# nianticlabs/simplerecon

Hardware: AMD Instinct MI355X
Metric: depth frames/sec (640x480, 7 src views, 64 planes) (higher is better)
Workload: dtype f32

## Files before the change

### include/simplerecon_hip.h

```cpp
#ifndef SIMPLERECON_HIP_H_
#define SIMPLERECON_HIP_H_

#include <stddef.h>
#include <stdint.h>

#ifdef __cplusplus
extern "C" {
#endif

#define SR_OK 0
#define SR_ERR_INVALID_ARGUMENT 1
#define SR_ERR_UNSUPPORTED 2
#define SR_ERR_WORKSPACE_TOO_SMALL 3
#define SR_ERR_HIP_BASE 1000

enum {
  SR_OPT_MLP_SPLIT = 0, SR_OPT_WINO_SPLIT, SR_OPT_WINO_XCD, SR_OPT_WINO_NT, SR_OPT_WINO_KSPLIT, SR_OPT_CONV_WINO,
  SR_OPT_CONV_TILE, SR_OPT_CONV_KSPLIT, SR_OPT_PW_NT, SR_OPT_PW_KS, SR_OPT_PT_CFG, SR_OPT_PT_KS, SR_OPT_DOT_LDS,
  SR_OPT_DOT_LDS_G, SR_OPT_DOT_LDS_CULL, SR_OPT_DOT_LDS_CAP, SR_OPT_UPSAMPLE_QUAD, SR_OPT_POOL_STREAM,
  SR_OPT_MLP_TILE,
  SR_OPT_COUNT
};
int sr_option_count(void);
const char* sr_option_name(int id);
int sr_option_id(const char* name);
int sr_option_get(int id, int* value);
int sr_option_set(int id, int value, int* previous );
int sr_option_default(int id, int* value);

int sr_abi_version(void);

const char* sr_target_arch(void);


size_t sr_volume_workspace_bytes(int B, int K, int C, int h, int w);

int sr_volume_prepare(const float* src, const float* K_src, const float* T_src_cur,
                      const float* T_cur_src, int B, int K, int C, int h, int w, void* workspace,
                      size_t workspace_bytes, void* stream);

int sr_dot_volume_sweep(const float* cur, const float* invK_cur, const float* planes, int64_t ps_b,
                        int64_t ps_d, int64_t ps_y, int64_t ps_x, int B, int K, int C, int h, int w,
                        int D, float* out_cv, int64_t cv_sb, int64_t cv_sd, int64_t cv_sp,
// ... 39 lines not shown
                      int h, int w, int D, float* out_cv, int64_t cv_sb, int64_t cv_sd,
                      int64_t cv_sp, float* out_lowest, uint8_t* out_mask, void* workspace,
                      size_t workspace_bytes, void* stream);

int sr_warp_features_fwd(const float* src, const float* K_src, const float* T_src_cur,
                         const float* invK_cur, const float* planes, int64_t ps_b, int64_t ps_d,
                         int64_t ps_y, int64_t ps_x, int B, int K, int C, int h, int w, int Dp,
                         float* out_world, float* out_depths, float* out_warped, float* out_mask,
                         float* out_pix, void* workspace, size_t workspace_bytes, void* stream);

size_t sr_mlp_volume_workspace_bytes(int B, int K, int C, int h, int w, int hidden);

int sr_mlp_pack_weights(const float* W1, const float* b1, const float* W2, const float* b2,
                        const float* W3, const float* b3, int hidden, int B, int K, int C, int h, int w,
                        void* workspace, size_t workspace_bytes, void* stream);

int sr_mlp_volume_sweep(const float* cur, const float* invK_cur, const float* planes, int64_t ps_b,
                        int64_t ps_d, int64_t ps_y, int64_t ps_x, float leaky_slope, int B, int K,
                        int C, int h, int w, int D, float* out_cv, int64_t cv_sb, int64_t cv_sd,
                        int64_t cv_sp, float* out_lowest, uint8_t* out_mask, void* workspace,
                        size_t workspace_bytes, void* stream);

int sr_mlp_volume_tile_shape(int h, int w, int* th, int* tw);

int sr_mlp_volume_fwd(const float* cur, const float* src, const float* K_src, const float* T_src_cur,
                      const float* T_cur_src, const float* invK_cur, const float* planes, int64_t ps_b,
                      int64_t ps_d, int64_t ps_y, int64_t ps_x, const float* W1, const float* b1,
                      const float* W2, const float* b2, const float* W3, const float* b3, int hidden,
                      float leaky_slope, int B, int K, int C, int h, int w, int D, float* out_cv,
                      int64_t cv_sb, int64_t cv_sd, int64_t cv_sp, float* out_lowest, uint8_t* out_mask,
                      int reserve_cus, void* workspace, size_t workspace_bytes, void* stream);


size_t sr_conv_packed_weight_floats(int Cout, int Cin, int ksize);

int sr_conv_pack_weights(const float* weight, int Cout, int Cin, int ksize, float* packed, void* stream);

int sr_conv2d_nhwc_fwd(const float* in, int64_t in_batch_stride, int in_pix_stride,
                       const float* packed_weight, const float* bias, const float* residual,
                       int64_t res_batch_stride, int res_pix_stride, float* out,
                       int64_t out_batch_stride, int out_pix_stride, int B, int H, int W, int Cin,
                       int Cout, int ksize, int stride, float leaky_slope, void* stream);

int sr_conv2d_replicate_nhwc_fwd(const float* in, int64_t in_batch_stride, int in_pix_stride,
                                 const float* packed_weight, const float* bias, const float* residual,
                                 int64_t res_batch_stride, int res_pix_stride, float* out,
// ... 422 lines not shown
```

### simplerecon_amd/_lib.py

```python
import contextlib
import ctypes as C
import os

import torch

_HERE = os.path.dirname(os.path.abspath(__file__))
LIB_PATH = os.environ.get("SR_HIP_LIBRARY") or os.path.join(_HERE, "libsimplerecon_hip.so")
ABI_VERSION = 3

_lib = None

_p = C.c_void_p
_i = C.c_int
_i64 = C.c_int64
_f = C.c_float
_sz = C.c_size_t

SIGNATURES = {
    "sr_abi_version": (_i, []),
    "sr_option_count": (_i, []),
    "sr_option_name": (C.c_char_p, [_i]),
    "sr_option_id": (_i, [C.c_char_p]),
    "sr_option_get": (_i, [_i, C.POINTER(C.c_int)]),
    "sr_option_set": (_i, [_i, _i, C.POINTER(C.c_int)]),
# ... 20 lines not shown
    "sr_conv16_wgrad_nhwc": (_i, [_p, _i64, _i, _p, _i64, _i, _p, _i, _i, _i, _i, _i, _i, _i, _i, _p, _sz, _p]),
    "sr_act_bwd_bias16_workspace_bytes": (_sz, [_i64, _i]),
    "sr_act_bwd_bias16_nhwc": (_i, [_p, _i, _p, _p, _p, _i64, _i, _f, _i, _p, _sz, _p]),
    "sr_pw_conv_tiled_workspace_bytes": (_sz, [_i, _i, _i]),
    "sr_pw_conv_tiled_plan": (_i, [_i, _i, _i, _i, _p, _p]),
    "sr_pw_conv_tiled_nhwc_fwd": (_i, [_p, _i, _p, _p, _p, _p, _i, _p, _i, _i, _i, _i, _i, _f, _p, _sz, _p]),
    "sr_pw_conv_supported": (_i, [_i, _i]),
    "sr_pw_conv_plan": (_i, [_i, _i, _i, _i, _p, _p]),
    "sr_pw_conv_nhwc_fwd": (_i, [_p, _i64, _i, _p, _p, _p, _p, _i64, _i, _p, _i64, _i, _i, _i, _i, _i, _f, _p]),
    "sr_backproject_fwd": (_i, [_p, _p, _p, _i, _i, _i, _p]),
    "sr_project3d_fwd": (_i, [_p, _p, _p, _p, _i, _i, _f, _p]),
    "sr_backproject_bwd": (_i, [_p, _p, _p, _i, _i, _i, _p]),
    "sr_project3d_bwd": (_i, [_p, _p, _p, _p, _p, _i, _i, _f, _p]),
    "sr_pose_distance_fwd": (_i, [_p, _p, _i, _p]),
    "sr_camera_rays_fwd": (_i, [_p, _p, _p, _i, _i, _i, _p]),
    "sr_selftest_rcp": (_i, [_p, _p, _p, _i, _p]),
    "sr_warp_features_fwd": (_i, [_p, _p, _p, _p, _p, _i64, _i64, _i64, _i64, _i, _i, _i, _i, _i, _i,
                                  _p, _p, _p, _p, _p, _p, _sz, _p]),
    "sr_mlp_volume_workspace_bytes": (_sz, [_i, _i, _i, _i, _i, _i]),
    "sr_mlp_pack_weights": (_i, [_p, _p, _p, _p, _p, _p, _i, _i, _i, _i, _i, _i, _p, _sz, _p]),
    "sr_mlp_volume_sweep": (_i, [_p, _p, _p, _i64, _i64, _i64, _i64, _f, _i, _i, _i, _i, _i, _i,
                                 _p, _i64, _i64, _i64, _p, _p, _p, _sz, _p]),
    "sr_mlp_volume_tile_shape": (_i, [_i, _i, C.POINTER(C.c_int), C.POINTER(C.c_int)]),
    "sr_mlp_volume_fwd": (_i, [_p, _p, _p, _p, _p, _p, _p, _i64, _i64, _i64, _i64, _p, _p, _p, _p, _p, _p, _i,
                               _f, _i, _i, _i, _i, _i, _i, _p, _i64, _i64, _i64, _p, _p, _i, _p, _sz, _p]),
    "sr_conv_packed_weight_floats": (_sz, [_i, _i, _i]),
    "sr_conv_pack_weights": (_i, [_p, _i, _i, _i, _p, _p]),
    "sr_conv2d_nhwc_fwd": (_i, [_p, _i64, _i, _p, _p, _p, _i64, _i, _p, _i64, _i, _i, _i, _i, _i, _i, _i, _i, _f, _p]),
    "sr_conv2d_replicate_nhwc_fwd": (_i, [_p, _i64, _i, _p, _p, _p, _i64, _i, _p, _i64, _i, _i, _i, _i, _i, _i, _i, _i,
                                          _f, _p]),
    "sr_conv2d_padded_nhwc_fwd": (_i, [_p, _i64, _i, _p, _p, _p, _i64, _i, _p, _i64, _i, _i, _i, _i, _i, _i, _i, _i,
                                       _i, _i, _i, _i, _f, _p]),
    "sr_dwconv3x3_pool_bands": (_i, [_i]),
    "sr_dwconv3x3_nhwc_fwd": (_i, [_p, _i64, _i, _p, _p, _p, _i64, _i, _p, _i, _i, _i, _i, _i, _i, _i, _i, _i, _f,
                                   _p]),
    "sr_add_nhwc_fwd": (_i, [_p, _i64, _i, _p, _i64, _i, _p, _i64, _i, _i, _i, _i, _i, _p]),
    "sr_se_scale_nhwc_fwd": (_i, [_p, _i, _p, _p, _p, _p, _p, _p, _i64, _i, _p, _i64, _i, _p, _i, _i, _i, _i, _i,
                                  _p]),
    "sr_se_gate_fwd": (_i, [_p, _i, _i, _p, _p, _p, _p, _p, _i, _i, _i, _p]),
    "sr_scale_channels_nhwc_fwd": (_i, [_p, _i64, _i, _p, _p, _i64, _i, _i, _i, _i, _i, _p]),
    "sr_dot_volume_bwd_scratch_bytes": (_sz, [_i, _i, _i, _i, _i]),
    "sr_dot_volume_bwd": (_i, [_p, _i64, _i64, _i64, _p, _p, _p, _i64, _i64, _i64, _i64, _i, _i, _i, _i, _i, _i, _p, _p,
                               _p, _sz, _p, _sz, _p]),
    "sr_mlp_volume_bwd_scratch_bytes": (_sz, [_i, _i, _i, _i, _i, _i]),
    "sr_mlp_volume_bwd": (_i, [_p, _i64, _i64, _i64, _p, _p, _p, _i64, _i64, _i64, _i64, _p, _p, _p, _p, _p, _f, _i, _i,
                               _i, _i, _i, _i, _i, _p, _p, _p, _p, _p, _p, _p, _p, _p, _sz, _p, _sz, _p]),
# ... 318 lines not shown
```

### simplerecon_amd/cost_volume.py

```python
import torch
from torch import Tensor, nn

from . import _lib
from .geometry import BackprojectDepth, Project3D
from .networks import MLP


def _autocast_on(device_type):
    try:
        return torch.is_autocast_enabled(device_type)
    except TypeError:
        return torch.is_autocast_enabled()


def _autocast_to_f32(*tensors):
    out = []
    for t in tensors:
        if isinstance(t, Tensor) and t.dtype in (torch.float16, torch.bfloat16) and _autocast_on(t.device.type):
            t = t.float()
        out.append(t)
    return out


class _DotVolumeFunction(torch.autograd.Function):
# ... 332 lines not shown
        lib = _lib.lib()
        vol, lowest, mask = self._alloc_outputs(b, h, w, dev, return_mask)
        if b == 0:
            return vol, lowest, mask
        params = [t.detach() for t in params]
        hidden = params[0].shape[0]
        nws = lib.sr_mlp_volume_workspace_bytes(b, k, c, h, w, hidden)
        ws = self._get_workspace(nws, dev)
        sb, sd, sp = self._volume_strides(vol)
        from . import ops
        cin, d = c * (k + 1) + 10 * k + 4, self.num_depth_bins
        record = lambda: ("sr_mlp_volume_fwd", 2.0 * (cin * hidden + hidden * hidden + hidden) * b * d * h * w, (), None)
        with _lib.SPLIT_GUARD:
            rc = ops._timed(
                dev, record, lib.sr_mlp_volume_fwd,
                _lib.ptr(cur), _lib.ptr(src), _lib.ptr(Ks), _lib.ptr(T), _lib.ptr(Tp), _lib.ptr(invK),
                _lib.ptr(planes), *planes.stride(), *[_lib.ptr(t) for t in params], hidden,
                0.01,
                b, k, c, h, w, d, _lib.ptr(vol), sb, sd, sp, _lib.ptr(lowest),
                _lib.ptr(mask), int(reserve_cus), _lib.ptr(ws), ws.numel(), _lib.stream_ptr(dev))
        _lib.check(rc, "sr_mlp_volume_fwd")
        return vol, lowest, mask

    def to_fast(self) -> "FastFeatureVolumeManager":
        manager = FastFeatureVolumeManager(self.matching_height, self.matching_width,
                                           num_depth_bins=self.num_depth_bins, mlp_channels=self.mlp_channels,
                                           matching_dim_size=self.matching_dim_size,
                                           num_source_views=self.num_source_views)
        manager.to(self.linear_ramp_1d11.device)
        manager.mlp = self.mlp
        manager.volume_memory_format = self.volume_memory_format
        return manager


class FastFeatureVolumeManager(FeatureVolumeManager):

    def warp_features(self, src_feats, src_extrinsics, src_Ks, cur_invK, depth_plane_bdhw, batch_size,
                      num_src_frames, num_feat_channels, uv_scale=None):
        world, depths, warped, mask, pix = self._warp(src_feats, src_extrinsics, src_Ks, cur_invK,
                                                      depth_plane_bdhw, True)
        b, dp = world.shape[:2]
        h, w = self.matching_height, self.matching_width
        world_bkd4hw = world.view(b, 1, dp, 4, h, w).expand(b, num_src_frames, dp, 4, h, w)
        return world_bkd4hw, depths, warped, mask, pix


# ... 20 lines not shown
```

### simplerecon_amd/csrc/sr_mlp_volume.hip

```cpp
#include <stdlib.h>
#include <string.h>

#include "sr_buffer.h"
#include "sr_view.h"

#define SR_HID 128
#define SR_VIEW_SLOTS 24
#define SR_INV_FIXED 20
#define SR_PLANE_CHUNK 8

static inline int sr_mlp_steps_var(int K) { return (SR_VIEW_SLOTS / 2) * K; }
static inline int sr_mlp_steps_inv(int K) { return (SR_INV_FIXED + 3 * K + 1) / 2; }
static inline int sr_mlp_steps1(int K) { return sr_mlp_steps_var(K) + sr_mlp_steps_inv(K); }
#define SR_MLP_STEPS2 65

static inline size_t sr_mlp_packed_floats(int K) { return (size_t)(sr_mlp_steps1(K) + SR_MLP_STEPS2) * 256 + 128 + 4; }

__global__ void sr_mlp_pack_kernel(const float* __restrict__ W1, const float* __restrict__ b1,
                                   const float* __restrict__ W2, const float* __restrict__ b2,
                                   const float* __restrict__ W3, const float* __restrict__ b3,
                                   float* __restrict__ packed, int K, int C) {
  const int steps_var = (SR_VIEW_SLOTS / 2) * K;
  const int steps1 = steps_var + (SR_INV_FIXED + 3 * K + 1) / 2;
  const int Cin = C * (K + 1) + 10 * K + 4;
// ... 46 lines not shown
    } else {
      v = b3[0];
    }
    packed[e] = v;
  }
}


struct SrMlpParams {
  const float* cur;
  const float* src_nhwc;
  const float* invK;
  const float* geom;
  const float* packed;
  SrPlanes planes;
  SrVolumeOut out;
  int B, K, h, w, D;
  int tiles;
  int tiles_x;
  int th_log2, tw_log2;
  int chunk, chunks;
  int vec_store;
  float inv_w, inv_h, slope;
};

__device__ __forceinline__ bool sr_mlp_lane_pixel(const SrMlpParams& p, int tile, int lane, int& y, int& x) {
  if (p.tiles_x) {
    const int ty = tile / p.tiles_x, tx = tile - ty * p.tiles_x;
    const int ly = (ty << p.th_log2) + (lane >> p.tw_log2);
    const int lx = (tx << p.tw_log2) + (lane & ((1 << p.tw_log2) - 1));
    y = min(ly, p.h - 1);
    x = min(lx, p.w - 1);
    return ly < p.h && lx < p.w;
  }
  const int N = p.h * p.w, pix = tile * 64 + lane;
  const int pc = min(pix, N - 1);
  y = pc / p.w;
  x = pc - y * p.w;
  return pix < N;
}

__device__ __forceinline__ void sr_swap_halves(float fa, float fb, float& bP, float& bQ) {
  auto r = __builtin_amdgcn_permlane32_swap(__float_as_uint(fa), __float_as_uint(fb), false, false);
  bP = __uint_as_float(r[0]);
  bQ = __uint_as_float(r[1]);
}

#define SR_MFMA(a, b, c) __builtin_amdgcn_mfma_f32_32x32x2f32((a), (b), (c), 0, 0, 0)

__device__ __forceinline__ void sr_l1_step(f32x16 (&acc)[2][4], const float4 wA, float fa, float fb) {
  float bP, bQ;
  sr_swap_halves(fa, fb, bP, bQ);
  acc[0][0] = SR_MFMA(wA.x, bP, acc[0][0]);
  acc[1][0] = SR_MFMA(wA.x, bQ, acc[1][0]);
  acc[0][1] = SR_MFMA(wA.y, bP, acc[0][1]);
  acc[1][1] = SR_MFMA(wA.y, bQ, acc[1][1]);
  acc[0][2] = SR_MFMA(wA.z, bP, acc[0][2]);
  acc[1][2] = SR_MFMA(wA.z, bQ, acc[1][2]);
  acc[0][3] = SR_MFMA(wA.w, bP, acc[0][3]);
  acc[1][3] = SR_MFMA(wA.w, bQ, acc[1][3]);
}

// ... 29 lines not shown
  const int steps1 = steps_var + (SR_INV_FIXED + 3 * p.K + 1) / 2;
  const float4* gW1 = reinterpret_cast<const float4*>(p.packed);
  const float4* gW1inv = gW1 + (size_t)steps_var * 64;
  const float4* gW2 = gW1 + (size_t)steps1 * 64;
  const float* gW3 = p.packed + (size_t)(steps1 + SR_MLP_STEPS2) * 256;

  for (int i = threadIdx.x; i < 129; i += blockDim.x) lds[i] = gW3[i];
  constexpr int W2_FLOATS = W2_LDS ? SR_MLP_STEPS2 * 256 : 0;
  if (W2_LDS) {
    float4* l4 = reinterpret_cast<float4*>(lds + SR_LDS_W3_FLOATS);
    for (int i = threadIdx.x; i < SR_MLP_STEPS2 * 64; i += blockDim.x) l4[i] = gW2[i];
  }
  if (W1_LDS) {
    float4* l4 = reinterpret_cast<float4*>(lds + SR_LDS_W3_FLOATS + W2_FLOATS);
    for (int i = threadIdx.x; i < steps_var * 64; i += blockDim.x) l4[i] = gW1[i];
  }
  __syncthreads();
  const float4* W1p = W1_LDS ? reinterpret_cast<const float4*>(lds + SR_LDS_W3_FLOATS + W2_FLOATS) : gW1;

  const int N = p.h * p.w;
  const long nunits = (long)p.B * p.tiles * p.chunks;
  constexpr int WPB = 4;
  const int wid = __builtin_amdgcn_readfirstlane(threadIdx.x >> 6);
  long wave0 = (long)blockIdx.x * WPB + wid;
  long nwaves = (long)gridDim.x * WPB;
  long unit_end = nunits;
  if ((gridDim.x & 7) == 0) {
    const long u8 = (nunits + 7) / 8;
    const int xcd = blockIdx.x & 7;
    nwaves = (long)(gridDim.x >> 3) * WPB;
    wave0 = xcd * u8 + (long)(blockIdx.x >> 3) * WPB + wid;
    unit_end = min(nunits, (xcd + 1) * u8);
  }
  const int half = lane >> 5;

  const int rot = (int)max(1L, nwaves / p.chunks);
  for (long unit = wave0; unit < unit_end; unit += nwaves) {
    const long tb = unit / p.chunks;
    const int chunk = (int)((unit % p.chunks + tb / rot) % p.chunks);
    const int tile = (int)(tb % p.tiles);
    const int b = (int)(tb / p.tiles);
    const int j0 = chunk * p.chunk, j1 = min(p.D, j0 + p.chunk);
    int y, x;
    const bool in_image = sr_mlp_lane_pixel(p, tile, lane, y, x);
    const int pc = y * p.w + x;
    const int pix = in_image ? pc : -1;
    const bool active = pix >= 0;
    const float* plane_ptr = p.planes.ptr + b * p.planes.sb + y * p.planes.sy + x * p.planes.sx;
    const float* geom_b = p.geom + (size_t)b * p.K * SR_GEOM_STRIDE;
    const float* src_b = p.src_nhwc + (size_t)b * p.K * N * C;

    float cur[C];
#pragma unroll
    for (int c = 0; c < C; ++c) cur[c] = p.cur[((size_t)b * C + c) * N + pc];

    float r0, r1, r2;
    {
#pragma clang fp contract(off)
      const float* iK = p.invK + 16 * (size_t)b;
      const float px = (float)x + 0.5f, py = (float)y + 0.5f;
      r0 = iK[0] * px + iK[1] * py + iK[2];
      r1 = iK[4] * px + iK[5] * py + iK[6];
      r2 = iK[8] * px + iK[9] * py + iK[10];
    }
    float cr0, cr1, cr2, crn0, crn1, crn2;
    {
#pragma clang fp contract(off)
      const float d0 = plane_ptr[0];
      const float X0 = d0 * r0, X1 = d0 * r1, X2 = d0 * r2;
      const float cden = fmaxf(sqrtf((X0 * X0 + X1 * X1) + X2 * X2), 1e-12f);
      cr0 = X0 / cden; cr1 = X1 / cden; cr2 = X2 / cden;
      const float n1 = fmaxf(sqrtf((cr0 * cr0 + cr1 * cr1) + cr2 * cr2), 1e-5f);
      crn0 = cr0 / n1; crn1 = cr1 / n1; crn2 = cr2 / n1;
    }

    f32x16 hc[2][4];
#pragma unroll
    for (int g = 0; g < 2; ++g)
#pragma unroll
      for (int m = 0; m < 4; ++m)
#pragma unroll
        for (int r = 0; r < 16; ++r) hc[g][m][r] = 0.0f;
    {
      const float4* wi = gW1inv + lane;
#pragma unroll
      for (int t = 0; t < 8; ++t) sr_l1_step(hc, wi[t * 64], cur[2 * t], cur[2 * t + 1]);
      sr_l1_step(hc, wi[8 * 64], cr0, cr1);
      sr_l1_step(hc, wi[9 * 64], cr2, 1.0f);
      const int npose = 3 * p.K;
#pragma unroll 1
      for (int u = 0; u < npose; u += 2) {
        const int ka = u / 3, ia = u - 3 * ka, kb = (u + 1) / 3, ib = (u + 1) - 3 * kb;
        const float fa = geom_b[ka * SR_GEOM_STRIDE + 15 + ia];
        const float fb = (u + 1 < npose) ? geom_b[kb * SR_GEOM_STRIDE + 15 + ib] : 0.0f;
        sr_l1_step(hc, wi[(size_t)(10 + (u >> 1)) * 64], fa, fb);
      }
    }

    SrSample smp;
    float4 taps[16];
    float X0, X1, X2, d;
    bool any_depth, any_bounds;
    float gt0, gt1, gt2;
    auto project_view = [&](int k) -> bool {
      const float* g = geom_b + k * SR_GEOM_STRIDE;
      gt0 = g[12]; gt1 = g[13]; gt2 = g[14];
      sr_project_sample(g, X0, X1, X2, p.h, p.w, p.inv_w, p.inv_h, smp);
      return __builtin_amdgcn_ballot_w64(active & smp.any_tap) == 0;
    };
    auto load_taps = [&](int k) {
      const float* img = src_b + (size_t)k * N * C;
      const float4* t_nw = reinterpret_cast<const float4*>(img + (size_t)smp.o_nw * C);
      const float4* t_ne = reinterpret_cast<const float4*>(img + (size_t)smp.o_ne * C);
      const float4* t_sw = reinterpret_cast<const float4*>(img + (size_t)smp.o_sw * C);
      const float4* t_se = reinterpret_cast<const float4*>(img + (size_t)smp.o_se * C);
#pragma unroll
      for (int i = 0; i < 4; ++i) {
        taps[i] = t_nw[i]; taps[4 + i] = t_ne[i]; taps[8 + i] = t_sw[i]; taps[12 + i] = t_se[i];
      }
    };
    float rv0, rv1, rv2, rsd, rdot;
#define SR_RAY_A_T(o, t0, t1, t2, kview)                                                      \
    {                                                                                         \
      _Pragma("clang fp contract(off)")                                                       \
      rv0 = X0 - (t0); rv1 = X1 - (t1); rv2 = X2 - (t2);                                       \
      rsd = fmaxf(sqrtf((rv0 * rv0 + rv1 * rv1) + rv2 * rv2), 1e-12f);                         \
      (o)[23] = ((kview) == 0) ? d : 0.0f;       \
    }
#define SR_RAY_A(o, g, kview) SR_RAY_A_T(o, (g)[12], (g)[13], (g)[14], kview)
#define SR_RAY_A0(o, kview) SR_RAY_A_T(o, gt0, gt1, gt2, kview)
#define SR_RAY_B(o)                                                                           \
// ... 33 lines not shown
      (o)[17] = smp.zp;                                    \
      (o)[18] = front ? rdot : 0.0f;                 \
    }
#define SR_DOT_DEAD(o)   \
    {                                                                                         \
      const bool front = smp.zp > 0.0f;                                                       \
      any_depth |= front;                                                                     \
      any_bounds |= sr_in_bounds(smp, p.h, p.w);                                              \
      (o)[16] = front ? 1.0f : 0.0f;                                                          \
      (o)[17] = smp.zp;                                                                       \
      (o)[18] = 0.0f;                                                                         \
    }
#define SR_SB __builtin_amdgcn_sched_barrier(0);

    constexpr bool CST_LDS = !W1_LDS;
    const int cst_base = SR_LDS_W3_FLOATS + W2_FLOATS +
                         wid * (SR_PLANE_CHUNK * 64);
    float cst[SR_PLANE_CHUNK];
#pragma unroll
    for (int q = 0; q < SR_PLANE_CHUNK; ++q) cst[q] = 0.0f;
#pragma unroll 1
    for (int j = j0; j < j1; ++j) {
      d = plane_ptr[j * p.planes.sd];
      {
#pragma clang fp contract(off)
        X0 = d * r0; X1 = d * r1; X2 = d * r2;
      }
      any_depth = false; any_bounds = false;
      f32x16 acc[2][4];
      float f[SR_VIEW_SLOTS], fn[SR_VIEW_SLOTS];

      bool dc = project_view(0), dn;
      if (!dc) {
        load_taps(0);
        SR_RAY_A0(f, 0) SR_RAY_B(f) SR_RAY_C(f)
        SR_INTERP2(f, 0, 0) SR_INTERP2(f, 0, 1) SR_INTERP2(f, 1, 0) SR_INTERP2(f, 1, 1)
        SR_INTERP2(f, 2, 0) SR_INTERP2(f, 2, 1) SR_INTERP2(f, 3, 0) SR_INTERP2(f, 3, 1)
        SR_DOT(f)
      } else {
        SR_RAY_A0(f, 0) SR_RAY_B(f) SR_RAY_C(f)
        SR_DOT_DEAD(f)
        f[0] = f[1] = 0.0f;
      }
#define SR_STEP(t)                                           \
        wN = wk[((t) + 1 < VS ? (t) + 1 : (t)) * 64];       \
        sr_l1_step(acc, wA, f[2 * (t)], f[2 * (t) + 1]);     \
        wA = wN;
#define SR_IF_LIVE(ND, x) if (!(ND)) { x }
#define SR_VIEW_BODY(FIRST, CD, ND)                                                    \
        {                                                                              \
// ... 111 lines not shown
        }
      }
      if (active) {
        if (!p.vec_store) p.out.cv[b * p.out.sb + j * p.out.sd + (int64_t)pix * p.out.sp] = cost;
        if (j == p.D - 1 && p.out.mask) p.out.mask[(size_t)b * N + pix] = (uint8_t)(any_depth && any_bounds);
      }
    }
    if (p.vec_store && active) {
      float* row = p.out.cv + b * p.out.sb + (int64_t)pix * p.out.sp + j0;
      if (CST_LDS) {
#pragma unroll
        for (int q = 0; q < SR_PLANE_CHUNK; ++q) cst[q] = lds[cst_base + q * 64 + lane];
      }
#pragma unroll
      for (int q = 0; q < SR_PLANE_CHUNK; q += 4) {
        if (j0 + q + 4 <= j1) *reinterpret_cast<float4*>(row + q) = make_float4(cst[q], cst[q + 1], cst[q + 2], cst[q + 3]);
        else {
#pragma unroll
          for (int i = 0; i < 4; ++i)
            if (j0 + q + i < j1) row[q + i] = cst[q + i];
        }
      }
    }
  }
}


template <int FMT> struct SrSplitFmt;
template <> struct SrSplitFmt<1> {
  typedef __bf16 e2 __attribute__((ext_vector_type(2)));
  typedef __bf16 e8 __attribute__((ext_vector_type(8)));
  static __device__ __forceinline__ void split(float a, float b, unsigned& hi, unsigned& lo) {
    const sr_f2v v = {a, b};
    hi = __builtin_bit_cast(unsigned, __builtin_convertvector(v, e2));
    const sr_f2v v0 = {__uint_as_float(hi << 16), __uint_as_float(hi & 0xffff0000u)};
    lo = __builtin_bit_cast(unsigned, __builtin_convertvector(v - v0, e2));
  }
  static __device__ __forceinline__ f32x16 mfma(sr_u4 a, sr_u4 b, f32x16 c) {
    return __builtin_amdgcn_mfma_f32_32x32x16_bf16(__builtin_bit_cast(e8, a), __builtin_bit_cast(e8, b), c, 0, 0, 0);
  }
};
template <> struct SrSplitFmt<2> {
  typedef _Float16 e2 __attribute__((ext_vector_type(2)));
  typedef _Float16 e8 __attribute__((ext_vector_type(8)));
  static __device__ __forceinline__ void split(float a, float b, unsigned& hi, unsigned& lo) {
    const sr_f2v v = {a, b};
// ... 365 lines not shown
  const int b = blockIdx.y;
  if (pix >= N) return;
  const int y = pix / w, x = pix - y * w;
  const float* c = cv + b * sb + (int64_t)pix * sp;
  float best = c[0];
  int bj = 0;
  int j = 1;
  for (; j + 8 <= D; j += 8) {
    float v[8];
#pragma unroll
    for (int u = 0; u < 8; ++u) v[u] = c[(int64_t)(j + u) * sd];
#pragma unroll
    for (int u = 0; u < 8; ++u)
      if (v[u] > best || (v[u] != v[u] && best == best)) { best = v[u]; bj = j + u; }
  }
  for (; j < D; ++j) {
    const float v = c[(int64_t)j * sd];
    if (v > best || (v != v && best == best)) { best = v; bj = j; }
  }
  lowest[(size_t)b * N + pix] = planes.ptr[b * planes.sb + bj * planes.sd + y * planes.sy + x * planes.sx];
}


extern "C" size_t sr_mlp_volume_workspace_bytes(int B, int K, int C, int h, int w, int hidden) {
  (void)hidden;
  if (B < 0 || K < 0) return 0;
  return sr_volume_workspace_bytes(B, K, C, h, w) + sr_align_up(sr_mlp_packed_floats(K) * sizeof(float), 256) + 256;
}

extern "C" int sr_mlp_volume_tile_shape(int h, int w, int* th, int* tw) {
  if (h <= 0 || w <= 0 || !th || !tw) return SR_ERR_INVALID_ARGUMENT;
  const int mode = sr_opt(SR_OPT_MLP_TILE);
  if (mode < 0 || mode > 4) return SR_ERR_INVALID_ARGUMENT;
  *th = 1; *tw = 64;
  if (mode >= 2) { *th = 1 << (mode - 1); *tw = 64 >> (mode - 1); }
  if (mode == 0) {
    const int64_t flat = ((int64_t)h * w + 63) / 64;
    for (int t = 8; t >= 2; t >>= 1) {
      const int64_t tiles = (int64_t)((h + t - 1) / t) * ((w + 64 / t - 1) / (64 / t));
      if (100 * tiles <= 101 * flat) { *th = t; *tw = 64 / t; break; }
    }
  }
  return SR_OK;
}

static float* sr_ws_packed(void* workspace, int B, int K, int C, int h, int w) {
  return (float*)sr_align_up((size_t)workspace + sr_volume_workspace_bytes(B, K, C, h, w), 256);
}

static int sr_mlp_volume_sweep_reserved(const float* cur, const float* invK_cur, const float* planes, int64_t ps_b,
                                        int64_t ps_d, int64_t ps_y, int64_t ps_x, float leaky_slope, int B, int K,
                                        int C, int h, int w, int D, float* out_cv, int64_t cv_sb, int64_t cv_sd,
                                        int64_t cv_sp, float* out_lowest, uint8_t* out_mask, int reserve_cus,
                                        void* workspace, size_t workspace_bytes, void* stream_) {
  if (B < 0 || K <= 0 || C <= 0 || h <= 0 || w <= 0 || D <= 0) return SR_ERR_INVALID_ARGUMENT;
  if (B == 0) return SR_OK;
  if (!cur || !invK_cur || !planes || !out_cv || !workspace) return SR_ERR_INVALID_ARGUMENT;
  if (C != 16) return SR_ERR_UNSUPPORTED;
  if (!(leaky_slope > 0.0f && leaky_slope < 1.0f)) return SR_ERR_UNSUPPORTED;
  if (workspace_bytes < sr_mlp_volume_workspace_bytes(B, K, C, h, w, SR_HID)) return SR_ERR_WORKSPACE_TOO_SMALL;
  hipStream_t stream = (hipStream_t)stream_;
  const int N = h * w;

  SrMlpParams p;
  p.cur = cur; p.src_nhwc = sr_ws_src_nhwc(workspace, B, K); p.invK = invK_cur; p.geom = sr_ws_geom(workspace);
  p.packed = sr_ws_packed(workspace, B, K, C, h, w);
  p.planes = {planes, ps_b, ps_d, ps_y, ps_x};
  p.out = {out_cv, cv_sb, cv_sd, cv_sp, out_lowest, out_mask};
  p.B = B; p.K = K; p.h = h; p.w = w; p.D = D;
  int th, tw;
  if (sr_mlp_volume_tile_shape(h, w, &th, &tw)) return SR_ERR_INVALID_ARGUMENT;
  p.th_log2 = __builtin_ctz(th); p.tw_log2 = __builtin_ctz(tw);
  p.tiles_x = th == 1 ? 0 : (w + tw - 1) / tw;
  p.tiles = th == 1 ? (N + 63) / 64 : p.tiles_x * ((h + th - 1) / th);
  p.inv_w = (float)(1.0 / (double)w);
  p.inv_h = (float)(1.0 / (double)h);
  p.slope = leaky_slope;

  int cus = sr_device_cus();
  if (reserve_cus > 0 && cus - reserve_cus >= 8) cus -= reserve_cus;
  const long waves = 4L * cus;
  double best_cost = 1e30;
  int best = 1;
  for (int c = SR_PLANE_CHUNK; c >= 1; c >>= 1) {
    const long units = (long)B * p.tiles * ((D + c - 1) / c);
    const long rounds = (units + waves - 1) / waves;
    const double cost = (double)rounds * (c * 1192.0 + 168.0);
    if (cost < best_cost) { best_cost = cost; best = c; }
  }
  p.chunk = best;
  p.chunks = (D + best - 1) / best;
  p.vec_store = (cv_sd == 1) && (p.chunk % 4 == 0) && sr_rows_aligned(out_cv, cv_sb, cv_sp, 15, 4);
  const long nunits = (long)B * p.tiles * p.chunks;
  const int blocks = (int)((nunits + 3) / 4 < cus ? (nunits + 3) / 4 : cus);
  const size_t w3_bytes = SR_LDS_W3_FLOATS * sizeof(float);
  const size_t w1_bytes = (size_t)sr_mlp_steps_var(K) * 1024;
  const size_t w2_bytes = (size_t)SR_MLP_STEPS2 * 1024;
  const size_t lds_max = 160 * 1024;
  const int split = sr_mlp_split_mode();
  if (split < 0) return SR_ERR_INVALID_ARGUMENT;
  if (split) {
    const size_t bytes = ((size_t)SR_SPL_TAB + SR_SPL_W2_WORDS + (size_t)K * SR_SPL_VIEW_WORDS) * 4;
    if (bytes > lds_max) return SR_ERR_UNSUPPORTED;
    const void* fn = split == 1 ? (const void*)sr_mlp_volume_split_kernel<1> : (const void*)sr_mlp_volume_split_kernel<2>;
    if (hipError_t e = sr_allow_lds(fn, bytes)) return sr_hip_rc(e);
    if (split == 1) hipLaunchKernelGGL((sr_mlp_volume_split_kernel<1>), dim3(blocks), dim3(256), bytes, stream, p);
    else hipLaunchKernelGGL((sr_mlp_volume_split_kernel<2>), dim3(blocks), dim3(256), bytes, stream, p);
    int rc = sr_hip_rc(hipGetLastError());
    if (rc) return rc;
    if (out_lowest) rc = sr_launch_argmax_planes(out_cv, cv_sb, cv_sd, cv_sp, p.planes, B, h, w, D, out_lowest, stream);
    return rc;
  }
#define SR_MLP_LAUNCH(L1, L2, BYTES)                                                                              \
  {                                                                                                               \
           \
    if (hipError_t e = sr_allow_lds((const void*)sr_mlp_volume_kernel<L1, L2>, (BYTES))) return sr_hip_rc(e);     \
    hipLaunchKernelGGL((sr_mlp_volume_kernel<L1, L2>), dim3(blocks), dim3(256), (BYTES), stream, p);              \
  }
  if (w1_bytes + w2_bytes + w3_bytes <= lds_max) SR_MLP_LAUNCH(true, true, w1_bytes + w2_bytes + w3_bytes)
  else if (w1_bytes + w3_bytes <= lds_max) SR_MLP_LAUNCH(true, false, w1_bytes + w3_bytes)
  else SR_MLP_LAUNCH(false, true, w2_bytes + w3_bytes + 4 * SR_PLANE_CHUNK * 64 * sizeof(float))
#undef SR_MLP_LAUNCH
  int rc = sr_hip_rc(hipGetLastError());
  if (rc) return rc;
  if (out_lowest) rc = sr_launch_argmax_planes(out_cv, cv_sb, cv_sd, cv_sp, p.planes, B, h, w, D, out_lowest, stream);
  return rc;
}

extern "C" int sr_mlp_volume_sweep(const float* cur, const float* invK_cur, const float* planes, int64_t ps_b,
                                   int64_t ps_d, int64_t ps_y, int64_t ps_x, float leaky_slope, int B, int K,
                                   int C, int h, int w, int D, float* out_cv, int64_t cv_sb, int64_t cv_sd,
                                   int64_t cv_sp, float* out_lowest, uint8_t* out_mask, void* workspace,
                                   size_t workspace_bytes, void* stream_) {
  return sr_mlp_volume_sweep_reserved(cur, invK_cur, planes, ps_b, ps_d, ps_y, ps_x, leaky_slope, B, K, C, h, w, D, out_cv,
                                      cv_sb, cv_sd, cv_sp, out_lowest, out_mask, 0, workspace, workspace_bytes, stream_);
}
// ... 20 lines not shown
  return sr_hip_rc(hipGetLastError());
}

extern "C" int sr_mlp_volume_fwd(const float* cur, const float* src, const float* K_src, const float* T_src_cur,
                                 const float* T_cur_src, const float* invK_cur, const float* planes, int64_t ps_b,
                                 int64_t ps_d, int64_t ps_y, int64_t ps_x, const float* W1, const float* b1,
                                 const float* W2, const float* b2, const float* W3, const float* b3, int hidden,
                                 float leaky_slope, int B, int K, int C, int h, int w, int D, float* out_cv,
                                 int64_t cv_sb, int64_t cv_sd, int64_t cv_sp, float* out_lowest, uint8_t* out_mask,
                                 int reserve_cus, void* workspace, size_t workspace_bytes, void* stream_) {
  if (B < 0 || K <= 0 || C <= 0 || h <= 0 || w <= 0 || D <= 0 || reserve_cus < 0) return SR_ERR_INVALID_ARGUMENT;
  if (B == 0) return SR_OK;
  if (!T_cur_src) return SR_ERR_INVALID_ARGUMENT;
  if (hidden != SR_HID || C != 16) return SR_ERR_UNSUPPORTED;
  if (workspace_bytes < sr_mlp_volume_workspace_bytes(B, K, C, h, w, hidden)) return SR_ERR_WORKSPACE_TOO_SMALL;
  int rc = sr_volume_prepare(src, K_src, T_src_cur, T_cur_src, B, K, C, h, w, workspace, workspace_bytes, stream_);
  if (rc) return rc;
  rc = sr_mlp_pack_weights(W1, b1, W2, b2, W3, b3, hidden, B, K, C, h, w, workspace, workspace_bytes, stream_);
  if (rc) return rc;
  return sr_mlp_volume_sweep_reserved(cur, invK_cur, planes, ps_b, ps_d, ps_y, ps_x, leaky_slope, B, K, C, h, w, D, out_cv,
                                      cv_sb, cv_sd, cv_sp, out_lowest, out_mask, reserve_cus, workspace, workspace_bytes,
                                      stream_);
}
```

### simplerecon_amd/csrc/sr_options.hip

```cpp
#include <atomic>
#include <map>
#include <mutex>
#include <utility>
#include <stdlib.h>
#include <string.h>

#include "sr_common.h"

namespace {

struct OptDef { const char* name; int dflt; int kind; };
const OptDef kDefs[SR_OPT_COUNT] = {
    {"SR_MLP_SPLIT", 0, 1},       {"SR_WINO_SPLIT", 0, 1},     {"SR_WINO_XCD", 1, 0},        {"SR_WINO_NT", 0, 0},
    {"SR_WINO_KSPLIT", 0, 0},     {"SR_CONV_WINO", 1, 0},      {"SR_CONV_TILE", 0, 0},       {"SR_CONV_KSPLIT", 1, 0},
    {"SR_PW_NT", 0, 0},           {"SR_PW_KS", 0, 0},          {"SR_PT_CFG", -1, 0},         {"SR_PT_KS", 0, 0},
    {"SR_DOT_LDS", 1, 0},         {"SR_DOT_LDS_G", 0, 0},      {"SR_DOT_LDS_CULL", 1, 0},    {"SR_DOT_LDS_CAP", 634, 0},
    {"SR_UPSAMPLE_QUAD", 1, 0},   {"SR_POOL_STREAM", 1, 0},    {"SR_MLP_TILE", 0, 2},
};
std::atomic<int> g_val[SR_OPT_COUNT];
std::once_flag g_once;

int parse(const OptDef& d, const char* e) {
  if (d.kind == 1) {
    if (!e || !*e || !strcmp(e, "0") || !strcmp(e, "off") || !strcmp(e, "fp32")) return 0;
    if (!strcmp(e, "bf16")) return 1;
    if (!strcmp(e, "f16") || !strcmp(e, "fp16")) return 2;
    return -1;
  }
  if (d.kind == 2) {
    static const char* const names[] = {"auto", "flat", "2x32", "4x16", "8x8"};
    if (!e || !*e) return d.dflt;
    for (int i = 0; i < 5; ++i)
      if (!strcmp(e, names[i])) return i;
    return -1;
  }
  return (e && *e) ? atoi(e) : d.dflt;
}

void init() {
  for (int i = 0; i < SR_OPT_COUNT; ++i) {
// ... 69 lines not shown
```

Measured before the change: 325.6.

## Balance MLP cost-volume work by sorting units on predicted dead-view count

Adds a pre-pass that counts, for each (batch, tile, plane-chunk) unit, how many source views project entirely out of bounds, then bucket-sorts units per XCD group by that cost. The MLP sweep kernel takes this order and walks it in serpentine fashion across rounds, so expensive and cheap units are spread evenly across waves. The aim is to cut load imbalance and tail time in the persistent sweep. In exchange it adds two extra kernel launches, a projection pass over every plane and view, and more workspace. It is enabled by default through a new option.

```diff
diff --git a/include/simplerecon_hip.h b/include/simplerecon_hip.h
--- a/include/simplerecon_hip.h
+++ b/include/simplerecon_hip.h
@@ -18,7 +18,7 @@
   SR_OPT_MLP_SPLIT = 0, SR_OPT_WINO_SPLIT, SR_OPT_WINO_XCD, SR_OPT_WINO_NT, SR_OPT_WINO_KSPLIT, SR_OPT_CONV_WINO,
   SR_OPT_CONV_TILE, SR_OPT_CONV_KSPLIT, SR_OPT_PW_NT, SR_OPT_PW_KS, SR_OPT_PT_CFG, SR_OPT_PT_KS, SR_OPT_DOT_LDS,
   SR_OPT_DOT_LDS_G, SR_OPT_DOT_LDS_CULL, SR_OPT_DOT_LDS_CAP, SR_OPT_UPSAMPLE_QUAD, SR_OPT_POOL_STREAM,
-  SR_OPT_MLP_TILE,
+  SR_OPT_MLP_TILE, SR_OPT_MLP_BALANCE,
   SR_OPT_COUNT
 };
 int sr_option_count(void);
@@ -104,6 +104,13 @@
                         size_t workspace_bytes, void* stream);
 
 int sr_mlp_volume_tile_shape(int h, int w, int* th, int* tw);
+
+int sr_mlp_volume_unit_order(const float* K_src, const float* T_src_cur, const float* T_cur_src,
+                             const float* invK_cur, const float* planes, int64_t ps_b, int64_t ps_d,
+                             int64_t ps_y, int64_t ps_x, int B, int K, int C, int h, int w, int D,
+                             int reserve_cus, int* out_dead, int* out_order, int64_t capacity,
+                             int64_t* out_units, int* out_groups, int* out_nw, int* out_chunk,
+                             void* workspace, size_t workspace_bytes, void* stream);
 
 int sr_mlp_volume_fwd(const float* cur, const float* src, const float* K_src, const float* T_src_cur,
                       const float* T_cur_src, const float* invK_cur, const float* planes, int64_t ps_b,
diff --git a/simplerecon_amd/_lib.py b/simplerecon_amd/_lib.py
--- a/simplerecon_amd/_lib.py
+++ b/simplerecon_amd/_lib.py
@@ -66,6 +66,8 @@
     "sr_mlp_volume_sweep": (_i, [_p, _p, _p, _i64, _i64, _i64, _i64, _f, _i, _i, _i, _i, _i, _i,
                                  _p, _i64, _i64, _i64, _p, _p, _p, _sz, _p]),
     "sr_mlp_volume_tile_shape": (_i, [_i, _i, C.POINTER(C.c_int), C.POINTER(C.c_int)]),
+    "sr_mlp_volume_unit_order": (_i, [_p, _p, _p, _p, _p, _i64, _i64, _i64, _i64, _i, _i, _i, _i, _i, _i, _i, _p, _p, _i64,
+                                      _p, _p, _p, _p, _p, _sz, _p]),
     "sr_mlp_volume_fwd": (_i, [_p, _p, _p, _p, _p, _p, _p, _i64, _i64, _i64, _i64, _p, _p, _p, _p, _p, _p, _i,
                                _f, _i, _i, _i, _i, _i, _i, _p, _i64, _i64, _i64, _p, _p, _i, _p, _sz, _p]),
     "sr_conv_packed_weight_floats": (_sz, [_i, _i, _i]),
diff --git a/simplerecon_amd/cost_volume.py b/simplerecon_amd/cost_volume.py
--- a/simplerecon_amd/cost_volume.py
+++ b/simplerecon_amd/cost_volume.py
@@ -378,6 +378,40 @@
         _lib.check(rc, "sr_mlp_volume_fwd")
         return vol, lowest, mask
 
+    def unit_order(self, src_extrinsics, src_poses, src_Ks, cur_invK, min_depth, max_depth, depth_planes_bdhw=None,
+                   reserve_cus=0):
+        import ctypes
+        import numpy as np
+        src_extrinsics, src_poses, src_Ks, cur_invK = _autocast_to_f32(src_extrinsics, src_poses, src_Ks, cur_invK)
+        for name, t in (("src_extrinsics", src_extrinsics), ("src_poses", src_poses), ("src_Ks", src_Ks),
+                        ("cur_invK", cur_invK)):
+            _lib.require_device_f32(name, t)
+        b, k = src_Ks.shape[:2]
+        c, h, w, d = self.matching_dim_size, self.matching_height, self.matching_width, self.num_depth_bins
+        planes = self._planes(b, min_depth, max_depth, depth_planes_bdhw)
+        dev = src_Ks.device
+        lib = _lib.lib()
+        Ks, T, Tp, invK = src_Ks.contiguous(), src_extrinsics.contiguous(), src_poses.contiguous(), cur_invK.contiguous()
+        ws = self._get_workspace(lib.sr_mlp_volume_workspace_bytes(b, k, c, h, w, self.mlp_channels[1]), dev)
+        units, groups, nw, chunk = ctypes.c_int64(0), ctypes.c_int(0), ctypes.c_int(0), ctypes.c_int(0)
+
+        def call(dead, order, capacity):
+            with _lib.on_device(dev):
+                rc = lib.sr_mlp_volume_unit_order(
+                    _lib.ptr(Ks), _lib.ptr(T), _lib.ptr(Tp), _lib.ptr(invK), _lib.ptr(planes), *planes.stride(), b, k, c,
+                    h, w, d, int(reserve_cus), dead, order, capacity, ctypes.addressof(units), ctypes.addressof(groups),
+                    ctypes.addressof(nw), ctypes.addressof(chunk), _lib.ptr(ws), ws.numel(), _lib.stream_ptr(dev))
+            _lib.check(rc, "sr_mlp_volume_unit_order")
+
+        call(None, None, 0)
+        out = {"units": units.value, "chunk": chunk.value, "chunks": -(-d // chunk.value), "nw": nw.value,
+               "groups": groups.value, "tiles": units.value // (b * -(-d // chunk.value)), "dead": None, "order": None}
+        if groups.value:
+            dead, order = np.empty(units.value, np.int32), np.full(units.value, -1, np.int32)
+            call(dead.ctypes.data, order.ctypes.data, units.value)
+            out["dead"], out["order"] = dead, order
+        return out
+
     def to_fast(self) -> "FastFeatureVolumeManager":
         manager = FastFeatureVolumeManager(self.matching_height, self.matching_width,
                                            num_depth_bins=self.num_depth_bins, mlp_channels=self.mlp_channels,
diff --git a/simplerecon_amd/csrc/sr_mlp_volume.hip b/simplerecon_amd/csrc/sr_mlp_volume.hip
--- a/simplerecon_amd/csrc/sr_mlp_volume.hip
+++ b/simplerecon_amd/csrc/sr_mlp_volume.hip
@@ -92,6 +92,7 @@
   int chunk, chunks;
   int vec_store;
   float inv_w, inv_h, slope;
+  const int* order;
 };
 
 __device__ __forceinline__ bool sr_mlp_lane_pixel(const SrMlpParams& p, int tile, int lane, int& y, int& x) {
@@ -108,6 +109,22 @@
   y = pc / p.w;
   x = pc - y * p.w;
   return pix < N;
+}
+
+__device__ __forceinline__ void sr_mlp_pixel_ray(const SrMlpParams& p, int b, int y, int x, float& r0, float& r1, float& r2) {
+#pragma clang fp contract(off)
+  const float* iK = p.invK + 16 * (size_t)b;
+  const float px = (float)x + 0.5f, py = (float)y + 0.5f;
+  r0 = iK[0] * px + iK[1] * py + iK[2];
+  r1 = iK[4] * px + iK[5] * py + iK[6];
+  r2 = iK[8] * px + iK[9] * py + iK[10];
+}
+__device__ __forceinline__ void sr_mlp_plane_point(float d, float r0, float r1, float r2, float& X0, float& X1, float& X2) {
+#pragma clang fp contract(off)
+  X0 = d * r0; X1 = d * r1; X2 = d * r2;
+}
+__device__ __forceinline__ bool sr_mlp_view_dead(bool active, const SrSample& smp) {
+  return __builtin_amdgcn_ballot_w64(active & smp.any_tap) == 0;
 }
 
 __device__ __forceinline__ void sr_swap_halves(float fa, float fb, float& bP, float& bQ) {
@@ -183,22 +200,34 @@
   const long nunits = (long)p.B * p.tiles * p.chunks;
   constexpr int WPB = 4;
   const int wid = __builtin_amdgcn_readfirstlane(threadIdx.x >> 6);
-  long wave0 = (long)blockIdx.x * WPB + wid;
+  long wl = (long)blockIdx.x * WPB + wid;
   long nwaves = (long)gridDim.x * WPB;
-  long unit_end = nunits;
+  long unit0 = 0, unit_end = nunits;
   if ((gridDim.x & 7) == 0) {
     const long u8 = (nunits + 7) / 8;
     const int xcd = blockIdx.x & 7;
     nwaves = (long)(gridDim.x >> 3) * WPB;
-    wave0 = xcd * u8 + (long)(blockIdx.x >> 3) * WPB + wid;
+    wl = (long)(blockIdx.x >> 3) * WPB + wid;
+    unit0 = xcd * u8;
     unit_end = min(nunits, (xcd + 1) * u8);
   }
   const int half = lane >> 5;
 
   const int rot = (int)max(1L, nwaves / p.chunks);
-  for (long unit = wave0; unit < unit_end; unit += nwaves) {
-    const long tb = unit / p.chunks;
-    const int chunk = (int)((unit % p.chunks + tb / rot) % p.chunks);
+  int round = 0;
+  for (long pos0 = unit0; pos0 < unit_end; pos0 += nwaves, ++round) {
+    const long pos = pos0 + ((p.order && (round & 1)) ? nwaves - 1 - wl : wl);
+    if (pos >= unit_end) continue;
+    long tb;
+    int chunk;
+    if (p.order) {
+      const int unit = __builtin_amdgcn_readfirstlane(p.order[pos]);
+      tb = unit / p.chunks;
+      chunk = unit - (int)tb * p.chunks;
+    } else {
+      tb = pos / p.chunks;
+      chunk = (int)((pos % p.chunks + tb / rot) % p.chunks);
+    }
     const int tile = (int)(tb % p.tiles);
     const int b = (int)(tb / p.tiles);
     const int j0 = chunk * p.chunk, j1 = min(p.D, j0 + p.chunk);
@@ -216,14 +245,7 @@
     for (int c = 0; c < C; ++c) cur[c] = p.cur[((size_t)b * C + c) * N + pc];
 
     float r0, r1, r2;
-    {
-#pragma clang fp contract(off)
-      const float* iK = p.invK + 16 * (size_t)b;
-      const float px = (float)x + 0.5f, py = (float)y + 0.5f;
-      r0 = iK[0] * px + iK[1] * py + iK[2];
-      r1 = iK[4] * px + iK[5] * py + iK[6];
-      r2 = iK[8] * px + iK[9] * py + iK[10];
-    }
+    sr_mlp_pixel_ray(p, b, y, x, r0, r1, r2);
     float cr0, cr1, cr2, crn0, crn1, crn2;
     {
 #pragma clang fp contract(off)
@@ -267,7 +289,7 @@
       const float* g = geom_b + k * SR_GEOM_STRIDE;
       gt0 = g[12]; gt1 = g[13]; gt2 = g[14];
       sr_project_sample(g, X0, X1, X2, p.h, p.w, p.inv_w, p.inv_h, smp);
-      return __builtin_amdgcn_ballot_w64(active & smp.any_tap) == 0;
+      return sr_mlp_view_dead(active, smp);
     };
     auto load_taps = [&](int k) {
       const float* img = src_b + (size_t)k * N * C;
@@ -347,10 +369,7 @@
 #pragma unroll 1
     for (int j = j0; j < j1; ++j) {
       d = plane_ptr[j * p.planes.sd];
-      {
-#pragma clang fp contract(off)
-        X0 = d * r0; X1 = d * r1; X2 = d * r2;
-      }
+      sr_mlp_plane_point(d, r0, r1, r2, X0, X1, X2);
       any_depth = false; any_bounds = false;
       f32x16 acc[2][4];
       float f[SR_VIEW_SLOTS], fn[SR_VIEW_SLOTS];
@@ -508,6 +527,86 @@
         }
       }
     }
+  }
+}
+
+
+__global__ __launch_bounds__(256) void sr_mlp_unit_cost_kernel(SrMlpParams p, int* __restrict__ dead) {
+  const int lane = threadIdx.x & 63;
+  const long nunits = (long)p.B * p.tiles * p.chunks;
+  const long unit = (long)blockIdx.x * 4 + __builtin_amdgcn_readfirstlane(threadIdx.x >> 6);
+  if (unit >= nunits) return;
+  const long tb = unit / p.chunks;
+  const int chunk = (int)(unit - tb * p.chunks);
+  const int tile = (int)(tb % p.tiles);
+  const int b = (int)(tb / p.tiles);
+  const int j0 = chunk * p.chunk, j1 = min(p.D, j0 + p.chunk);
+  int y, x;
+  const bool active = sr_mlp_lane_pixel(p, tile, lane, y, x);
+  const float* plane_ptr = p.planes.ptr + b * p.planes.sb + y * p.planes.sy + x * p.planes.sx;
+  const float* geom_b = p.geom + (size_t)b * p.K * SR_GEOM_STRIDE;
+  float r0, r1, r2;
+  sr_mlp_pixel_ray(p, b, y, x, r0, r1, r2);
+  int n = 0;
+  for (int j = j0; j < j1; ++j) {
+    float X0, X1, X2;
+    sr_mlp_plane_point(plane_ptr[j * p.planes.sd], r0, r1, r2, X0, X1, X2);
+    for (int k = 0; k < p.K; ++k) {
+      SrSample smp;
+      sr_project_sample(geom_b + k * SR_GEOM_STRIDE, X0, X1, X2, p.h, p.w, p.inv_w, p.inv_h, smp);
+      n += sr_mlp_view_dead(active, smp) ? 1 : 0;
+    }
+  }
+  if (lane == 0) dead[unit] = n;
+}
+
+#define SR_ORD_THREADS 128
+#define SR_ORD_ROW (SR_ORD_THREADS + 1)
+static inline size_t sr_mlp_order_lds_bytes(int nkey) { return (size_t)nkey * (SR_ORD_ROW + 1) * sizeof(int); }
+
+__global__ __launch_bounds__(SR_ORD_THREADS) void sr_mlp_unit_order_kernel(const int* __restrict__ dead,
+                                                                           int* __restrict__ order, long nunits,
+                                                                           int groups, int chunk, int chunks, int D, int K) {
+  extern __shared__ int ord_lds[];
+  const int nkey = chunk * K + 1;
+  int* hist = ord_lds;
+  int* base = ord_lds + nkey * SR_ORD_ROW;
+  const int t = threadIdx.x;
+  const long U = (nunits + groups - 1) / groups;
+  const long start = blockIdx.x * U, end = min(nunits, start + U);
+  if (start >= end) return;
+  const long per = (end - start + SR_ORD_THREADS - 1) / SR_ORD_THREADS;
+  const long i0 = min(end, start + t * per), i1 = min(end, i0 + per);
+  auto key_of = [&](long i) {
+    const int c = (int)(i % chunks);
+    const int lacking = chunk - (min(D, (c + 1) * chunk) - c * chunk);
+    return min(max(dead[i] + lacking * K, 0), nkey - 1);
+  };
+  for (int e = t; e < nkey * SR_ORD_ROW; e += SR_ORD_THREADS) hist[e] = 0;
+  __syncthreads();
+  for (long i = i0; i < i1; ++i) hist[key_of(i) * SR_ORD_ROW + t] += 1;
+  __syncthreads();
+  for (int key = t; key < nkey; key += SR_ORD_THREADS) {
+    int run = 0;
+    for (int s = 0; s < SR_ORD_THREADS; ++s) {
+      const int v = hist[key * SR_ORD_ROW + s];
+      hist[key * SR_ORD_ROW + s] = run;
+      run += v;
+    }
+    hist[key * SR_ORD_ROW + SR_ORD_THREADS] = run;
+  }
+  __syncthreads();
+  for (int key = t; key < nkey; key += SR_ORD_THREADS) {
+    int first = 0;
+    for (int q = 0; q < key; ++q) first += hist[q * SR_ORD_ROW + SR_ORD_THREADS];
+    base[key] = first;
+  }
+  __syncthreads();
+  for (long i = i0; i < i1; ++i) {
+    const int key = key_of(i);
+    const int at = base[key] + hist[key * SR_ORD_ROW + t];
+    hist[key * SR_ORD_ROW + t] += 1;
+    order[start + at] = (int)i;
   }
 }
 
@@ -919,10 +1018,23 @@
 }
 
 
+#define SR_MLP_BALANCE_PLANES 128
+static size_t sr_mlp_unit_capacity(int B, int h, int w) {
+  if (B <= 0 || h <= 0 || w <= 0) return 0;
+  size_t tiles = ((size_t)h * w + 63) / 64;
+  for (int t = 8; t >= 2; t >>= 1) {
+    const size_t n = (size_t)((h + t - 1) / t) * ((w + 64 / t - 1) / (64 / t));
+    if (n > tiles) tiles = n;
+  }
+  return (size_t)B * tiles * SR_MLP_BALANCE_PLANES;
+}
+static size_t sr_mlp_unit_table_bytes(int B, int h, int w) { return sr_align_up(sr_mlp_unit_capacity(B, h, w) * sizeof(int), 256); }
+
 extern "C" size_t sr_mlp_volume_workspace_bytes(int B, int K, int C, int h, int w, int hidden) {
   (void)hidden;
   if (B < 0 || K < 0) return 0;
-  return sr_volume_workspace_bytes(B, K, C, h, w) + sr_align_up(sr_mlp_packed_floats(K) * sizeof(float), 256) + 256;
+  return sr_volume_workspace_bytes(B, K, C, h, w) + sr_align_up(sr_mlp_packed_floats(K) * sizeof(float), 256) + 256 +
+         2 * sr_mlp_unit_table_bytes(B, h, w);
 }
 
 extern "C" int sr_mlp_volume_tile_shape(int h, int w, int* th, int* tw) {
@@ -943,6 +1055,65 @@
 
 static float* sr_ws_packed(void* workspace, int B, int K, int C, int h, int w) {
   return (float*)sr_align_up((size_t)workspace + sr_volume_workspace_bytes(B, K, C, h, w), 256);
+}
+static int* sr_ws_unit_dead(void* workspace, int B, int K, int C, int h, int w) {
+  return (int*)((char*)sr_ws_packed(workspace, B, K, C, h, w) + sr_align_up(sr_mlp_packed_floats(K) * sizeof(float), 256));
+}
+static int* sr_ws_unit_order(void* workspace, int B, int K, int C, int h, int w) {
+  return (int*)((char*)sr_ws_unit_dead(workspace, B, K, C, h, w) + sr_mlp_unit_table_bytes(B, h, w));
+}
+
+struct SrMlpPlan {
+  int blocks;
+  long nunits;
+  int balance;
+  int groups, nw;
+};
+static int sr_mlp_plan(SrMlpParams& p, int B, int K, int C, int h, int w, int D, int reserve_cus, void* workspace,
+                       SrMlpPlan& plan) {
+  const int N = h * w;
+  p.B = B; p.K = K; p.h = h; p.w = w; p.D = D;
+  int th, tw;
+  if (sr_mlp_volume_tile_shape(h, w, &th, &tw)) return SR_ERR_INVALID_ARGUMENT;
+  p.th_log2 = __builtin_ctz(th); p.tw_log2 = __builtin_ctz(tw);
+  p.tiles_x = th == 1 ? 0 : (w + tw - 1) / tw;
+  p.tiles = th == 1 ? (N + 63) / 64 : p.tiles_x * ((h + th - 1) / th);
+  p.inv_w = (float)(1.0 / (double)w);
+  p.inv_h = (float)(1.0 / (double)h);
+
+  int cus = sr_device_cus();
+  if (reserve_cus > 0 && cus - reserve_cus >= 8) cus -= reserve_cus;
+  const long waves = 4L * cus;
+  double best_cost = 1e30;
+  int best = 1;
+  for (int c = SR_PLANE_CHUNK; c >= 1; c >>= 1) {
+    const long units = (long)B * p.tiles * ((D + c - 1) / c);
+    const long rounds = (units + waves - 1) / waves;
+    const double cost = (double)rounds * (c * 1192.0 + 168.0);
+    if (cost < best_cost) { best_cost = cost; best = c; }
+  }
+  p.chunk = best;
+  p.chunks = (D + best - 1) / best;
+  plan.nunits = (long)B * p.tiles * p.chunks;
+  plan.blocks = (int)((plan.nunits + 3) / 4 < cus ? (plan.nunits + 3) / 4 : cus);
+  plan.groups = (plan.blocks & 7) == 0 ? 8 : 1;
+  plan.nw = plan.blocks / plan.groups * 4;
+
+  const int mode = sr_opt(SR_OPT_MLP_BALANCE);
+  if (mode < 0 || mode > 1) return SR_ERR_INVALID_ARGUMENT;
+  plan.balance = mode == 1 && D <= SR_MLP_BALANCE_PLANES && (size_t)plan.nunits <= sr_mlp_unit_capacity(B, h, w) &&
+                 plan.nunits <= 0x7fffffffL && sr_mlp_order_lds_bytes(p.chunk * K + 1) <= 160 * 1024;
+  p.order = plan.balance ? sr_ws_unit_order(workspace, B, K, C, h, w) : nullptr;
+  return SR_OK;
+}
+
+static int sr_mlp_launch_unit_order(const SrMlpParams& p, const SrMlpPlan& plan, int* dead, hipStream_t stream) {
+  hipLaunchKernelGGL(sr_mlp_unit_cost_kernel, dim3((unsigned)((plan.nunits + 3) / 4)), dim3(256), 0, stream, p, dead);
+  const size_t bytes = sr_mlp_order_lds_bytes(p.chunk * p.K + 1);
+  if (hipError_t e = sr_allow_lds((const void*)sr_mlp_unit_order_kernel, bytes)) return sr_hip_rc(e);
+  hipLaunchKernelGGL(sr_mlp_unit_order_kernel, dim3(plan.groups), dim3(SR_ORD_THREADS), bytes, stream, dead,
+                     const_cast<int*>(p.order), plan.nunits, plan.groups, p.chunk, p.chunks, p.D, p.K);
+  return sr_hip_rc(hipGetLastError());
 }
 
 static int sr_mlp_volume_sweep_reserved(const float* cur, const float* invK_cur, const float* planes, int64_t ps_b,
@@ -957,39 +1128,17 @@
   if (!(leaky_slope > 0.0f && leaky_slope < 1.0f)) return SR_ERR_UNSUPPORTED;
   if (workspace_bytes < sr_mlp_volume_workspace_bytes(B, K, C, h, w, SR_HID)) return SR_ERR_WORKSPACE_TOO_SMALL;
   hipStream_t stream = (hipStream_t)stream_;
-  const int N = h * w;
 
   SrMlpParams p;
   p.cur = cur; p.src_nhwc = sr_ws_src_nhwc(workspace, B, K); p.invK = invK_cur; p.geom = sr_ws_geom(workspace);
   p.packed = sr_ws_packed(workspace, B, K, C, h, w);
   p.planes = {planes, ps_b, ps_d, ps_y, ps_x};
   p.out = {out_cv, cv_sb, cv_sd, cv_sp, out_lowest, out_mask};
-  p.B = B; p.K = K; p.h = h; p.w = w; p.D = D;
-  int th, tw;
-  if (sr_mlp_volume_tile_shape(h, w, &th, &tw)) return SR_ERR_INVALID_ARGUMENT;
-  p.th_log2 = __builtin_ctz(th); p.tw_log2 = __builtin_ctz(tw);
-  p.tiles_x = th == 1 ? 0 : (w + tw - 1) / tw;
-  p.tiles = th == 1 ? (N + 63) / 64 : p.tiles_x * ((h + th - 1) / th);
-  p.inv_w = (float)(1.0 / (double)w);
-  p.inv_h = (float)(1.0 / (double)h);
   p.slope = leaky_slope;
-
-  int cus = sr_device_cus();
-  if (reserve_cus > 0 && cus - reserve_cus >= 8) cus -= reserve_cus;
-  const long waves = 4L * cus;
-  double best_cost = 1e30;
-  int best = 1;
-  for (int c = SR_PLANE_CHUNK; c >= 1; c >>= 1) {
-    const long units = (long)B * p.tiles * ((D + c - 1) / c);
-    const long rounds = (units + waves - 1) / waves;
-    const double cost = (double)rounds * (c * 1192.0 + 168.0);
-    if (cost < best_cost) { best_cost = cost; best = c; }
-  }
-  p.chunk = best;
-  p.chunks = (D + best - 1) / best;
+  SrMlpPlan plan;
+  if (int rc = sr_mlp_plan(p, B, K, C, h, w, D, reserve_cus, workspace, plan)) return rc;
   p.vec_store = (cv_sd == 1) && (p.chunk % 4 == 0) && sr_rows_aligned(out_cv, cv_sb, cv_sp, 15, 4);
-  const long nunits = (long)B * p.tiles * p.chunks;
-  const int blocks = (int)((nunits + 3) / 4 < cus ? (nunits + 3) / 4 : cus);
+  const int blocks = plan.blocks;
   const size_t w3_bytes = SR_LDS_W3_FLOATS * sizeof(float);
   const size_t w1_bytes = (size_t)sr_mlp_steps_var(K) * 1024;
   const size_t w2_bytes = (size_t)SR_MLP_STEPS2 * 1024;
@@ -1008,7 +1157,9 @@
     if (out_lowest) rc = sr_launch_argmax_planes(out_cv, cv_sb, cv_sd, cv_sp, p.planes, B, h, w, D, out_lowest, stream);
     return rc;
   }
-#define SR_MLP_LAUNCH(L1, L2, BYTES)                                                                              \
+  if (plan.balance)
+    if (int rc = sr_mlp_launch_unit_order(p, plan, sr_ws_unit_dead(workspace, B, K, C, h, w), stream)) return rc;
+#define SR_MLP_LAUNCH(L1, L2, BYTES)                                                                             \
   {                                                                                                               \
            \
     if (hipError_t e = sr_allow_lds((const void*)sr_mlp_volume_kernel<L1, L2>, (BYTES))) return sr_hip_rc(e);     \
@@ -1075,3 +1226,36 @@
                                       cv_sb, cv_sd, cv_sp, out_lowest, out_mask, reserve_cus, workspace, workspace_bytes,
                                       stream_);
 }
+
+extern "C" int sr_mlp_volume_unit_order(const float* K_src, const float* T_src_cur, const float* T_cur_src,
+                                        const float* invK_cur, const float* planes, int64_t ps_b, int64_t ps_d,
+                                        int64_t ps_y, int64_t ps_x, int B, int K, int C, int h, int w, int D,
+                                        int reserve_cus, int* out_dead, int* out_order, int64_t capacity,
+                                        int64_t* out_units, int* out_groups, int* out_nw, int* out_chunk,
+                                        void* workspace, size_t workspace_bytes, void* stream_) {
+  if (B <= 0 || K <= 0 || h <= 0 || w <= 0 || D <= 0 || reserve_cus < 0 || capacity < 0) return SR_ERR_INVALID_ARGUMENT;
+  if (!K_src || !T_src_cur || !T_cur_src || !invK_cur || !planes || !workspace) return SR_ERR_INVALID_ARGUMENT;
+  if (C != 16) return SR_ERR_UNSUPPORTED;
+  if (workspace_bytes < sr_mlp_volume_workspace_bytes(B, K, C, h, w, SR_HID)) return SR_ERR_WORKSPACE_TOO_SMALL;
+  hipStream_t stream = (hipStream_t)stream_;
+  SrMlpParams p = {};
+  p.invK = invK_cur; p.geom = sr_ws_geom(workspace);
+  p.planes = {planes, ps_b, ps_d, ps_y, ps_x};
+  SrMlpPlan plan;
+  if (int rc = sr_mlp_plan(p, B, K, C, h, w, D, reserve_cus, workspace, plan)) return rc;
+  if (out_units) *out_units = plan.nunits;
+  if (out_groups) *out_groups = plan.balance ? plan.groups : 0;
+  if (out_nw) *out_nw = plan.nw;
+  if (out_chunk) *out_chunk = p.chunk;
+  if (!plan.balance || (!out_dead && !out_order)) return SR_OK;
+  if (capacity < plan.nunits) return SR_ERR_INVALID_ARGUMENT;
+  if (int rc = sr_launch_geom(K_src, T_src_cur, T_cur_src, sr_ws_geom(workspace), B * K, stream)) return rc;
+  int* dead = sr_ws_unit_dead(workspace, B, K, C, h, w);
+  if (int rc = sr_mlp_launch_unit_order(p, plan, dead, stream)) return rc;
+  const size_t bytes = (size_t)plan.nunits * sizeof(int);
+  if (out_dead)
+    if (hipError_t e = hipMemcpyAsync(out_dead, dead, bytes, hipMemcpyDeviceToHost, stream)) return sr_hip_rc(e);
+  if (out_order)
+    if (hipError_t e = hipMemcpyAsync(out_order, p.order, bytes, hipMemcpyDeviceToHost, stream)) return sr_hip_rc(e);
+  return sr_hip_rc(hipStreamSynchronize(stream));
+}
diff --git a/simplerecon_amd/csrc/sr_options.hip b/simplerecon_amd/csrc/sr_options.hip
--- a/simplerecon_amd/csrc/sr_options.hip
+++ b/simplerecon_amd/csrc/sr_options.hip
@@ -16,6 +16,7 @@
     {"SR_PW_NT", 0, 0},           {"SR_PW_KS", 0, 0},          {"SR_PT_CFG", -1, 0},         {"SR_PT_KS", 0, 0},
     {"SR_DOT_LDS", 1, 0},         {"SR_DOT_LDS_G", 0, 0},      {"SR_DOT_LDS_CULL", 1, 0},    {"SR_DOT_LDS_CAP", 634, 0},
     {"SR_UPSAMPLE_QUAD", 1, 0},   {"SR_POOL_STREAM", 1, 0},    {"SR_MLP_TILE", 0, 2},
+    {"SR_MLP_BALANCE", 1, 0},
 };
 std::atomic<int> g_val[SR_OPT_COUNT];
 std::once_flag g_once;
```

New measurement: 327.5 (median of 6 runs). Within noise of the previous version (+0.6%).
